# megvii-research/CVPR2023-UniDistill

Hardware: AMD Instinct MI355X
Metric: distill-train samples/sec (nuScenes frame); bev_pool+voxelize HBM GB/s (higher is better)
Workload: dtype f32; 1 GPU; camera_exp_distill_lidar: student+teacher distillation step, 6 cams 256x704, 30000-pt cloud, 40 GT boxes, fwd+bwd+AdamW; batch_per_gpu=4, global_batch=4, parallelism=dp1, layout=channels-last dense convs, executor=eager+DDP, strict_no_library_fallthrough=True, wgrad_stream=on, ranks=1, dist_backend=none (single process)

## Files before the change

cvpr2023-unidistill_amd/csrc/conv2d_f32_wino_wgrad.hip:

```cpp
#include "ud_common.h"
#include "ud_prof.h"
#include <cstdlib>
#include <type_traits>

namespace {

typedef float f32x4 __attribute__((ext_vector_type(4)));

constexpr int kST = 8;
constexpr int kBufBytes = 2 * 16 * kST * 64 * 4;
constexpr int kVHalf = 16 * kST * 64 * 4;

struct WwGeom {
  int B, H, W, Cin, Cout, TX, TY;
  long long ntiles;
  int nstages, sps;
};

__global__ __launch_bounds__(512) void k_wino_wgrad_f32(const float* __restrict__ x, const float* __restrict__ dy,
                                                        float* __restrict__ partial, WwGeom gm) {
  extern __shared__ __attribute__((aligned(16))) char smem[];
  const int tid = threadIdx.x, lane = tid & 63;
  const int wave = __builtin_amdgcn_readfirstlane(tid >> 6);
  const int g = lane >> 4, li = lane & 15;
  const int n0 = blockIdx.y * 64, c0 = blockIdx.z * 64;
  const int s_begin = blockIdx.x * gm.sps, s_end = min(gm.nstages, s_begin + gm.sps);
  const bool cok = c0 + lane < gm.Cin, nok = n0 + lane < gm.Cout;

  float rx[2][16], rd[2][4];
  const unsigned xlane = (unsigned)min(c0 + lane, gm.Cin - 1), dlane = (unsigned)min(n0 + lane, gm.Cout - 1);
  unsigned xmask[2] = {0, 0}, dmask[2] = {0, 0};
  int tb, tty, ttx;
  {
    const long long t = (long long)s_begin * kST + wave;
    const int per = gm.TX * gm.TY;
    tb = (int)(t / per);
    const int rem = (int)(t - (long long)tb * per);
    tty = rem / gm.TX, ttx = rem - tty * gm.TX;
  }
  unsigned rowx[4], colx[4], rowd[2], cold[2], xm_cur = 0, dm_cur = 0;
  bool st_interior = false, wrapped = true;
  const bool xfull = c0 + 64 <= gm.Cin, dfull = n0 + 64 <= gm.Cout;
  auto load_part = [&](auto set_c, int part) {
    constexpr int S = decltype(set_c)::value;
    if (part == 0) {
      const bool inter = tb < gm.B && ttx >= 1 && 2 * ttx + 2 < gm.W;
      if (st_interior && inter && !wrapped) {
#pragma unroll
        for (int j = 0; j < 4; ++j) colx[j] += 2 * kST * (unsigned)gm.Cin;
        cold[0] += 2 * kST * (unsigned)gm.Cout;
        cold[1] += 2 * kST * (unsigned)gm.Cout;
      } else {
        const int tv = tb < gm.B ? 1 : 0;
        const unsigned img = (unsigned)(tv ? tb : 0) * gm.H * gm.W;
        unsigned rmask = 0, cmask = 0, rowoff[4], coloff[4];
#pragma unroll
        for (int i = 0; i < 4; ++i) {
          const int gy = 2 * tty - 1 + i, gx = 2 * ttx - 1 + i;
          rmask |= (unsigned)((gy >= 0) & (gy < gm.H) & tv) << i;
          cmask |= (unsigned)((gx >= 0) & (gx < gm.W)) << i;
          rowoff[i] = img + (unsigned)min(max(gy, 0), gm.H - 1) * gm.W;
          coloff[i] = (unsigned)min(max(gx, 0), gm.W - 1);
          rowx[i] = rowoff[i] * (unsigned)gm.Cin;
          colx[i] = coloff[i] * (unsigned)gm.Cin;
        }
        rowd[0] = rowoff[1] * (unsigned)gm.Cout, rowd[1] = rowoff[2] * (unsigned)gm.Cout;
        cold[0] = coloff[1] * (unsigned)gm.Cout, cold[1] = coloff[2] * (unsigned)gm.Cout;
        xm_cur = dm_cur = 0;
#pragma unroll
        for (int i = 0; i < 4; ++i) xm_cur |= ((rmask >> i) & 1) ? cmask << (4 * i) : 0u;
#pragma unroll
        for (int a = 0; a < 2; ++a) dm_cur |= ((rmask >> (a + 1)) & 1) ? ((cmask >> 1) & 3u) << (2 * a) : 0u;
      }
      st_interior = inter;
      xmask[S] = xm_cur, dmask[S] = dm_cur;
    } else if (part < 3) {
#pragma unroll
      for (int i = 2 * (part - 1); i < 2 * (part - 1) + 2; ++i)
#pragma unroll
        for (int j = 0; j < 4; ++j) rx[S][4 * i + j] = x[rowx[i] + colx[j] + xlane];
    } else {
#pragma unroll
      for (int a = 0; a < 2; ++a)
#pragma unroll
        for (int q = 0; q < 2; ++q) rd[S][2 * a + q] = dy[rowd[a] + cold[q] + dlane];
      ttx += kST;
      wrapped = false;
      while (ttx >= gm.TX) {
        ttx -= gm.TX;
        wrapped = true;
        if (++tty == gm.TY) tty = 0, ++tb;
      }
    }
  };
  auto load_raw = [&](auto set_c) {
#pragma unroll
    for (int part = 0; part < 4; ++part) load_part(set_c, part);
  };
  float td[4][4];
  auto transform_part = [&](auto set_c, int buf, int part) {
    constexpr int S = decltype(set_c)::value;
    float* D = reinterpret_cast<float*>(smem + buf * kBufBytes) + wave * 64 + lane;
    float* V = reinterpret_cast<float*>(smem + buf * kBufBytes + kVHalf) + wave * 64 + lane;
    if (part == 0) {
      if (!(dfull && dmask[S] == 0xFu)) {
#pragma unroll
        for (int k = 0; k < 4; ++k) rd[S][k] = (nok && ((dmask[S] >> k) & 1)) ? rd[S][k] : 0.f;
      }
      const float* r = rd[S];
      const float z[4][2] = {{r[0], r[1]}, {r[0] + r[2], r[1] + r[3]}, {r[0] - r[2], r[1] - r[3]}, {-r[2], -r[3]}};
#pragma unroll
      for (int i = 0; i < 4; ++i) {
        D[(4 * i + 0) * 512] = z[i][0];
        D[(4 * i + 1) * 512] = z[i][0] + z[i][1];
        D[(4 * i + 2) * 512] = z[i][0] - z[i][1];
        D[(4 * i + 3) * 512] = -z[i][1];
      }
    } else if (part == 1) {
      if (!(xfull && xmask[S] == 0xFFFFu)) {
#pragma unroll
        for (int k = 0; k < 16; ++k) rx[S][k] = (cok && ((xmask[S] >> k) & 1)) ? rx[S][k] : 0.f;
      }
#pragma unroll
      for (int j = 0; j < 4; ++j) {
        td[0][j] = rx[S][j] - rx[S][8 + j];
        td[1][j] = rx[S][4 + j] + rx[S][8 + j];
        td[2][j] = rx[S][8 + j] - rx[S][4 + j];
        td[3][j] = rx[S][4 + j] - rx[S][12 + j];
      }
    } else {
#pragma unroll
      for (int i = 2 * (part - 2); i < 2 * (part - 2) + 2; ++i) {
        V[(4 * i + 0) * 512] = td[i][0] - td[i][2];
        V[(4 * i + 1) * 512] = td[i][1] + td[i][2];
        V[(4 * i + 2) * 512] = td[i][2] - td[i][1];
        V[(4 * i + 3) * 512] = td[i][1] - td[i][3];
      }
    }
  };
  auto transform = [&](auto set_c, int buf) {
#pragma unroll
    for (int part = 0; part < 4; ++part) transform_part(set_c, buf, part);
  };

  f32x4 acc[2][4][4];
#pragma unroll
  for (int fi = 0; fi < 2; ++fi)
#pragma unroll
    for (int a = 0; a < 4; ++a)
#pragma unroll
      for (int q = 0; q < 4; ++q) acc[fi][a][q] = (f32x4){0.f, 0.f, 0.f, 0.f};

  f32x4 qa[2], qb[2];
  const unsigned fbase = (2 * wave) * 2048 + g * 256 + li * 16;
#define UD_WW_LOADS(BUF, FI, K)                                                                                        \
  do {                                                                                                                 \
    asm volatile("ds_read_b128 %0, %1 offset:%2" : "=v"(qa[BUF]) : "v"(pf), "n"((FI) * 2048 + (K) * 1024));            \
    asm volatile("ds_read_b128 %0, %1 offset:%2" : "=v"(qb[BUF]) : "v"(pf), "n"(kVHalf + (FI) * 2048 + (K) * 1024));   \
  } while (0)
#define UD_WW_WAIT(BUF, N) asm volatile("s_waitcnt lgkmcnt(" #N ")" : "+v"(qa[BUF]), "+v"(qb[BUF]))

  using Set0 = std::integral_constant<int, 0>;
  using Set1 = std::integral_constant<int, 1>;
  const int nst = s_end - s_begin;
  if (nst > 0) {
    load_raw(Set0{});
    transform(Set0{}, 0);
    if (nst > 1) load_raw(Set1{});
  }
  auto stage = [&](auto par_c, int k) {
    constexpr int P = decltype(par_c)::value;
    using SetP = std::integral_constant<int, P>;
    using SetQ = std::integral_constant<int, P ^ 1>;
    asm volatile("s_waitcnt lgkmcnt(0)" ::: "memory");
    __syncthreads();
    const bool more = k + 1 < nst, more2 = k + 2 < nst;
    const unsigned pf = fbase + P * kBufBytes;
    UD_WW_LOADS(0, 0, 0);
#pragma unroll
    for (int st = 0; st < 4; ++st) {
      const int cur = st & 1;
      if (st + 1 < 4) {
        if (cur == 0) UD_WW_LOADS(1, (st + 1) >> 1, (st + 1) & 1); else UD_WW_LOADS(0, (st + 1) >> 1, (st + 1) & 1);
        if (cur == 0) UD_WW_WAIT(0, 2); else UD_WW_WAIT(1, 2);
      } else {
        UD_WW_WAIT(1, 0);
      }
      const int fi = st >> 1;
      const bool ride = (st == 0 && more2) || (st == 3 && more);
      if (ride) {
        __builtin_amdgcn_sched_barrier(0);
        if (st == 0) load_raw(SetP{}); else transform(SetQ{}, P ^ 1);
      }
#pragma unroll
      for (int a = 0; a < 4; ++a)
#pragma unroll
        for (int q = 0; q < 4; ++q)
          acc[fi][a][q] = __builtin_amdgcn_mfma_f32_16x16x4f32(qa[cur][a], qb[cur][q], acc[fi][a][q], 0, 0, 0);
      if (ride) {
#pragma unroll
        for (int i_ = 0; i_ < 16; ++i_) {
          __builtin_amdgcn_sched_group_barrier(0x008, 1, 0);
          if (st == 0) {
            __builtin_amdgcn_sched_group_barrier(0x006, 6, 0);
            __builtin_amdgcn_sched_group_barrier(0x020, 2, 0);
          } else {
            __builtin_amdgcn_sched_group_barrier(0x002, 6, 0);
            __builtin_amdgcn_sched_group_barrier(0x200, 2, 0);
          }
        }
        __builtin_amdgcn_sched_barrier(0);
      }
    }
  };
  for (int k = 0; k < nst; k += 2) {
    stage(Set0{}, k);
    if (k + 1 < nst) stage(Set1{}, k + 1);
  }
#undef UD_WW_LOADS
#undef UD_WW_WAIT
  const int c = c0 + 4 * li;
  if (c < gm.Cin) {
#pragma unroll
    for (int fi = 0; fi < 2; ++fi)
#pragma unroll
      for (int a = 0; a < 4; ++a)
#pragma unroll
        for (int r = 0; r < 4; ++r) {
          const int n = n0 + 4 * (4 * g + r) + a;
          if (n < gm.Cout)
            *reinterpret_cast<float4*>(partial + (((size_t)blockIdx.x * 16 + 2 * wave + fi) * gm.Cout + n) * gm.Cin + c) =
                make_float4(acc[fi][a][0][r], acc[fi][a][1][r], acc[fi][a][2][r], acc[fi][a][3][r]);
        }
  }
}

__global__ __launch_bounds__(256) void k_wino_wgrad_finish(const float* __restrict__ partial, int nslices, int Cout, int Cin,
                                                           float* __restrict__ dw) {
  __shared__ float4 M[16][16];
  const int cx = threadIdx.x & 15, f = threadIdx.x >> 4;
  const int n = blockIdx.x, c = blockIdx.y * 64 + cx * 4;
  float4 s = make_float4(0.f, 0.f, 0.f, 0.f);
  if (c < Cin)
    for (int sl = 0; sl < nslices; ++sl) {
      const float4 v = *reinterpret_cast<const float4*>(partial + (((size_t)sl * 16 + f) * Cout + n) * Cin + c);
      s.x += v.x; s.y += v.y; s.z += v.z; s.w += v.w;
    }
  M[f][cx] = s;
  __syncthreads();
  if (f < 9 && c < Cin) {
    const float GT[3][4] = {{1.f, 0.5f, 0.5f, 0.f}, {0.f, 0.5f, -0.5f, 0.f}, {0.f, 0.5f, 0.5f, 1.f}};
    const int ky = f / 3, kx = f - 3 * ky;
    float4 o = make_float4(0.f, 0.f, 0.f, 0.f);
#pragma unroll
    for (int i = 0; i < 4; ++i)
#pragma unroll
      for (int j = 0; j < 4; ++j) {
        const float k = GT[ky][i] * GT[kx][j];
        const float4 m = M[4 * i + j][cx];
        o.x += k * m.x; o.y += k * m.y; o.z += k * m.z; o.w += k * m.w;
      }
    *reinterpret_cast<float4*>(dw + ((size_t)n * 9 + f) * Cin + c) = o;
  }
}

struct WwPlan {
  int TX, TY, nstages, sps, nslices, nb, cb;
  long long ntiles;
};
WwPlan ww_plan(int B, int H, int W, int Cin, int Cout) {
  WwPlan p;
  p.TX = (W + 1) / 2, p.TY = (H + 1) / 2;
  p.ntiles = (long long)B * p.TX * p.TY;
  p.nstages = (int)((p.ntiles + kST - 1) / kST);
  p.nb = ud_div_up(Cout, 64), p.cb = ud_div_up(Cin, 64);
  int slices = 256 / (p.nb * p.cb);
  if (slices < 1) slices = 1;
  if (slices > p.nstages) slices = p.nstages;
  p.sps = ud_div_up(p.nstages, slices);
  p.nslices = ud_div_up(p.nstages, p.sps);
  return p;
}

}

extern "C" size_t ud_conv3x3_wino_wgrad_f32_workspace_bytes(int B, int H, int W, int Cin, int Cout) {
  if (B <= 0 || H <= 0 || W <= 0 || Cin <= 0 || Cout <= 0) return 0;
  const WwPlan p = ww_plan(B, H, W, Cin, Cout);
  return (size_t)p.nslices * 16 * Cout * Cin * sizeof(float);
}

extern "C" int ud_conv3x3_wino_wgrad_nhwc_f32(const float* x, const float* dy, float* dw, int B, int H, int W, int Cin,
                                              int Cout, void* workspace, size_t workspace_bytes, ud_stream_t stream_) {
  if (!x || !dy || !dw || !workspace || B <= 0 || H <= 0 || W <= 0 || Cin <= 0 || Cout <= 0) return UD_ERR_INVALID_ARG;
  if (Cin % 4 != 0 || Cout % 4 != 0) return UD_ERR_UNSUPPORTED;
  const WwPlan p = ww_plan(B, H, W, Cin, Cout);
  if (workspace_bytes < (size_t)p.nslices * 16 * Cout * Cin * sizeof(float)) return UD_ERR_WORKSPACE;
  if (p.nb > 65535 || p.cb > 65535 || (long long)B * H * W * Cin >= (1ll << 31) || (long long)B * H * W * Cout >= (1ll << 31))
    return UD_ERR_UNSUPPORTED;
  hipStream_t stream = (hipStream_t)stream_;
  static UdDeviceOnce attr_set;
  if (const int e = ud_allow_dyn_lds(attr_set, (int)(2 * kBufBytes), k_wino_wgrad_f32)) return e;
  UdProfScope prof("conv2d.k_wgrad_wino_f32", stream);
  float* partial = static_cast<float*>(workspace);
  WwGeom gm{B, H, W, Cin, Cout, p.TX, p.TY, p.ntiles, p.nstages, p.sps};
  k_wino_wgrad_f32<<<dim3(p.nslices, p.nb, p.cb), 512, 2 * kBufBytes, stream>>>(x, dy, partial, gm);
  UD_LAUNCH_CHECK();
  k_wino_wgrad_finish<<<dim3(Cout, ud_div_up(Cin, 64)), 256, 0, stream>>>(partial, p.nslices, Cout, Cin, dw);
  UD_LAUNCH_CHECK();
  return UD_OK;
}
```

Measured before the change: 68.96 samples/s.

## Apply Winograd output transform in wgrad kernel epilogue before slice reduction

Moves the Winograd G^T·M·G output transform from the separate finish kernel into the main wgrad kernel epilogue. The 16 accumulator planes are staged through LDS, transformed into 9 filter taps per slice, and written as partials. A generic slice-sum routine then reduces them into dw. This cuts partial-workspace traffic from 16 to 9 planes per slice and simplifies the reduction, at the cost of extra LDS passes and barriers in the epilogue.

```diff
diff --git a/cvpr2023-unidistill_amd/csrc/conv2d_f32_wino_wgrad.hip b/cvpr2023-unidistill_amd/csrc/conv2d_f32_wino_wgrad.hip
--- a/cvpr2023-unidistill_amd/csrc/conv2d_f32_wino_wgrad.hip
+++ b/cvpr2023-unidistill_amd/csrc/conv2d_f32_wino_wgrad.hip
@@ -1,5 +1,6 @@
 #include "ud_common.h"
 #include "ud_prof.h"
+#include "ud_reduce.h"
 #include <cstdlib>
 #include <type_traits>
 
@@ -219,48 +220,44 @@
   }
 #undef UD_WW_LOADS
 #undef UD_WW_WAIT
-  const int c = c0 + 4 * li;
-  if (c < gm.Cin) {
+  float* E = reinterpret_cast<float*>(smem);
+  const int enl = tid >> 4, ec = c0 + 4 * (tid & 15);
+#pragma unroll
+  for (int p = 0; p < 2; ++p) {
+    __syncthreads();
 #pragma unroll
     for (int fi = 0; fi < 2; ++fi)
 #pragma unroll
-      for (int a = 0; a < 4; ++a)
+      for (int ai = 0; ai < 2; ++ai)
 #pragma unroll
         for (int r = 0; r < 4; ++r) {
-          const int n = n0 + 4 * (4 * g + r) + a;
-          if (n < gm.Cout)
-            *reinterpret_cast<float4*>(partial + (((size_t)blockIdx.x * 16 + 2 * wave + fi) * gm.Cout + n) * gm.Cin + c) =
-                make_float4(acc[fi][a][0][r], acc[fi][a][1][r], acc[fi][a][2][r], acc[fi][a][3][r]);
+          const int a = 2 * p + ai;
+          *reinterpret_cast<float4*>(E + ((2 * wave + fi) * 32 + 8 * g + 2 * r + ai) * 64 + 4 * li) =
+              make_float4(acc[fi][a][0][r], acc[fi][a][1][r], acc[fi][a][2][r], acc[fi][a][3][r]);
         }
-  }
-}
-
-__global__ __launch_bounds__(256) void k_wino_wgrad_finish(const float* __restrict__ partial, int nslices, int Cout, int Cin,
-                                                           float* __restrict__ dw) {
-  __shared__ float4 M[16][16];
-  const int cx = threadIdx.x & 15, f = threadIdx.x >> 4;
-  const int n = blockIdx.x, c = blockIdx.y * 64 + cx * 4;
-  float4 s = make_float4(0.f, 0.f, 0.f, 0.f);
-  if (c < Cin)
-    for (int sl = 0; sl < nslices; ++sl) {
-      const float4 v = *reinterpret_cast<const float4*>(partial + (((size_t)sl * 16 + f) * Cout + n) * Cin + c);
-      s.x += v.x; s.y += v.y; s.z += v.z; s.w += v.w;
+    __syncthreads();
+    const int n = n0 + 16 * (enl >> 3) + 4 * ((enl >> 1) & 3) + 2 * p + (enl & 1);
+    if (n < gm.Cout && ec < gm.Cin) {
+      f32x4 u[4][3];
+#pragma unroll
+      for (int i = 0; i < 4; ++i) {
+        f32x4 m[4];
+#pragma unroll
+        for (int j = 0; j < 4; ++j) m[j] = *reinterpret_cast<const f32x4*>(E + ((4 * i + j) * 32 + enl) * 64 + 4 * (tid & 15));
+        const f32x4 hs = 0.5f * (m[1] + m[2]);
+        u[i][0] = m[0] + hs;
+        u[i][1] = 0.5f * (m[1] - m[2]);
+        u[i][2] = hs + m[3];
+      }
+      float* o = partial + (((size_t)blockIdx.x * gm.Cout + n) * 9) * gm.Cin + ec;
+#pragma unroll
+      for (int kx = 0; kx < 3; ++kx) {
+        const f32x4 hs = 0.5f * (u[1][kx] + u[2][kx]);
+        *reinterpret_cast<f32x4*>(o + (size_t)kx * gm.Cin) = u[0][kx] + hs;
+        *reinterpret_cast<f32x4*>(o + (size_t)(3 + kx) * gm.Cin) = 0.5f * (u[1][kx] - u[2][kx]);
+        *reinterpret_cast<f32x4*>(o + (size_t)(6 + kx) * gm.Cin) = hs + u[3][kx];
+      }
     }
-  M[f][cx] = s;
-  __syncthreads();
-  if (f < 9 && c < Cin) {
-    const float GT[3][4] = {{1.f, 0.5f, 0.5f, 0.f}, {0.f, 0.5f, -0.5f, 0.f}, {0.f, 0.5f, 0.5f, 1.f}};
-    const int ky = f / 3, kx = f - 3 * ky;
-    float4 o = make_float4(0.f, 0.f, 0.f, 0.f);
-#pragma unroll
-    for (int i = 0; i < 4; ++i)
-#pragma unroll
-      for (int j = 0; j < 4; ++j) {
-        const float k = GT[ky][i] * GT[kx][j];
-        const float4 m = M[4 * i + j][cx];
-        o.x += k * m.x; o.y += k * m.y; o.z += k * m.z; o.w += k * m.w;
-      }
-    *reinterpret_cast<float4*>(dw + ((size_t)n * 9 + f) * Cin + c) = o;
   }
 }
 
@@ -287,7 +284,7 @@
 extern "C" size_t ud_conv3x3_wino_wgrad_f32_workspace_bytes(int B, int H, int W, int Cin, int Cout) {
   if (B <= 0 || H <= 0 || W <= 0 || Cin <= 0 || Cout <= 0) return 0;
   const WwPlan p = ww_plan(B, H, W, Cin, Cout);
-  return (size_t)p.nslices * 16 * Cout * Cin * sizeof(float);
+  return (size_t)p.nslices * 9 * Cout * Cin * sizeof(float);
 }
 
 extern "C" int ud_conv3x3_wino_wgrad_nhwc_f32(const float* x, const float* dy, float* dw, int B, int H, int W, int Cin,
@@ -295,7 +292,7 @@
   if (!x || !dy || !dw || !workspace || B <= 0 || H <= 0 || W <= 0 || Cin <= 0 || Cout <= 0) return UD_ERR_INVALID_ARG;
   if (Cin % 4 != 0 || Cout % 4 != 0) return UD_ERR_UNSUPPORTED;
   const WwPlan p = ww_plan(B, H, W, Cin, Cout);
-  if (workspace_bytes < (size_t)p.nslices * 16 * Cout * Cin * sizeof(float)) return UD_ERR_WORKSPACE;
+  if (workspace_bytes < (size_t)p.nslices * 9 * Cout * Cin * sizeof(float)) return UD_ERR_WORKSPACE;
   if (p.nb > 65535 || p.cb > 65535 || (long long)B * H * W * Cin >= (1ll << 31) || (long long)B * H * W * Cout >= (1ll << 31))
     return UD_ERR_UNSUPPORTED;
   hipStream_t stream = (hipStream_t)stream_;
@@ -306,7 +303,5 @@
   WwGeom gm{B, H, W, Cin, Cout, p.TX, p.TY, p.ntiles, p.nstages, p.sps};
   k_wino_wgrad_f32<<<dim3(p.nslices, p.nb, p.cb), 512, 2 * kBufBytes, stream>>>(x, dy, partial, gm);
   UD_LAUNCH_CHECK();
-  k_wino_wgrad_finish<<<dim3(Cout, ud_div_up(Cin, 64)), 256, 0, stream>>>(partial, p.nslices, Cout, Cin, dw);
-  UD_LAUNCH_CHECK();
-  return UD_OK;
-}
+  return ud_wgrad_sum(partial, p.nslices, (size_t)Cout * 9 * Cin, dw, stream);
+}
```

Result: no change. 68.95 samples/s (median of 2 runs) (-0.0%).
